# sleepybishop/nanorq

Measured on AMD Instinct MI355X. Metric: Gbit/s encode+decode, K=8192 T=1280, higher is better.
Workload: dtype u8

## Files before the change

__graft_entry__.py:

```python
import os
import sys

ROOT = os.path.dirname(os.path.abspath(__file__))
for p in (ROOT, os.path.join(ROOT, "tests")):
    if p not in sys.path:
        sys.path.insert(0, p)


def build():
    from nanorq_amd import build as nbuild
    nbuild.build_lib(verbose=True)
    nbuild.build_emu()
    nbuild.build_planner_emu()
    nbuild.build_ingest_emu()
    nbuild.build_emit_emu()
    nbuild.build_held_emu()
    nbuild.build_rxset_emu()
    nbuild.build_rxset_lists_emu()
    nbuild.build_txset_emu()
    nbuild.build_obj_emu()
    nbuild.build_shape_emu()
    nbuild.build_tools()
    import oracle
    oracle.build()
    if os.path.isfile("/root/reference/benchmark.c"):
        import subprocess
        subprocess.run(["make", "-s", "-C", os.path.join(ROOT, "oracle"), "_ref/benchmark_hip", "_ref/encode_hip", "_ref/decode_hip"],
                       check=True)
    import nanorq_amd
    nanorq_amd.lib()
    print("build ok:", nanorq_amd.lib_path())


def smoke():
    import numpy as np
# ... 29 lines not shown
```

nanorq_amd/binding.py:

```python
import ctypes as C
import os

import numpy as np

_HERE = os.path.dirname(os.path.abspath(__file__))
_LIB = None


class NrqError(RuntimeError):
    pass


class ObjParams(C.Structure):
    _fields_ = [("F", C.c_uint64)] + [(n, C.c_uint32) for n in
                                       ("T", "Al", "Z", "N", "Kt", "ZL", "KL", "KpL", "ZS", "KS", "KpS", "NL", "TL", "NS", "TS",
                                        "flags", "max_esi")] + [("oti_common", C.c_uint64), ("oti_specific", C.c_uint32)]

    def as_dict(self):
        return {n: getattr(self, n) for n, _ in self._fields_}


class CallStats(C.Structure):
    _fields_ = [("plan_ms", C.c_double), ("host_ms", C.c_double), ("strip_bytes", C.c_uint32),
                ("lds_bytes", C.c_uint32), ("grid", C.c_uint32), ("planner", C.c_uint32),
# ... 121 lines not shown
        L.nrq_rxset_decode.argtypes = [vp, ip, u32p]
    if hasattr(L, "nrq_txset_create"):
        L.nrq_txset_create.argtypes = [vp, C.c_uint32, C.POINTER(vp)]
        L.nrq_txset_destroy.argtypes = [vp]
        L.nrq_txset_destroy.restype = None
        L.nrq_txset_attach.argtypes = [vp, C.c_uint32, vp]
        L.nrq_txset_attach_obj.argtypes = [vp, C.c_uint32, vp]
        L.nrq_txset_detach.argtypes = [vp, C.c_uint32]
        L.nrq_txset_blocks.argtypes = [vp, u32p, u32p, C.c_uint32, u32p]
        L.nrq_txset_emit.argtypes = [vp, vp, vp, C.c_uint32, vp, sz, C.c_uint32, vp]
    u8pp = C.POINTER(C.POINTER(C.c_uint8))
    L.nrq_host_kconst_build.argtypes = [C.c_uint32, u8pp, u32p]
    L.nrq_host_plan_build.argtypes = [C.c_uint32, C.c_uint32, u32p, C.POINTER(C.c_uint8), u8pp, u32p]
    L.nrq_host_free.argtypes = [vp]
    L.nrq_host_free.restype = None
    _LIB = L
    return L


PARAM_NAMES = ("Kp", "J", "S", "H", "W", "L", "P", "P1", "U", "B")
PLAN_FIELDS = ("magic status K Kp J S H W L P P1 B M npiv u nlow r2 nfree nlev nrows pipe wpr "
               "npiv_pad n_xor_ops off_ops off_pivslot off_pivcol off_wt off_lowslot off_pivx off_fbits "
               "off_mh off_freex off_hinv off_colslot off_pivof off_uslot total_bytes reserved0 reserved1 fail_site "
               "off_augt lpr aug_stride nneed need_pad off_needslot off_wneed").split()


def params(K):
    out = (C.c_uint32 * 10)()
    if lib().nrq_params(K, out) != 0:
        raise ValueError("K out of range: %r" % (K,))
    return dict(zip(PARAM_NAMES, (int(x) for x in out)))


def _u32(a):
    return a.ctypes.data_as(C.POINTER(C.c_uint32))


def host_kconst(K):
    out = C.POINTER(C.c_uint8)()
    n = C.c_uint32()
    if lib().nrq_host_kconst_build(K, C.byref(out), C.byref(n)) != 0:
        raise NrqError("kconst build failed")
    buf = bytes(C.string_at(out, n.value))
    lib().nrq_host_free(out)
    return buf


# ... 664 lines not shown
```

nanorq_amd/build.py:

```python
import os
import shutil
import subprocess
import sys

HERE = os.path.dirname(os.path.abspath(__file__))
ROOT = os.path.dirname(HERE)
CSRC = os.path.join(HERE, "csrc")
LIB = os.path.join(HERE, "libnanorq_hip.so")
EMU = os.path.join(ROOT, "tests", "emu", "libsolve_emu.so")
PEMU = os.path.join(ROOT, "tests", "emu", "libplanner_emu.so")
IEMU = os.path.join(ROOT, "tests", "emu", "libingest_emu.so")
XEMU = os.path.join(ROOT, "tests", "emu", "libemit_emu.so")
OEMU = os.path.join(ROOT, "tests", "emu", "libobj_emu.so")
SEMU = os.path.join(ROOT, "tests", "emu", "libshape_emu.so")
HEMU = os.path.join(ROOT, "tests", "emu", "libheld_emu.so")
WEMU = os.path.join(ROOT, "tests", "emu", "libwant_emu.so")
REMU = os.path.join(ROOT, "tests", "emu", "librxset_emu.so")
LEMU = os.path.join(ROOT, "tests", "emu", "librxset_lists_emu.so")
TEMU = os.path.join(ROOT, "tests", "emu", "libtxset_emu.so")

HIP_SOURCES = ["nrq_device.hip"]
CXX_SOURCES = ["planner_host.cpp"]
C_SOURCES = ["nanorq_api.c", "io.c"]


def _hipcc():
    for c in (os.environ.get("HIPCC"), "/opt/rocm/bin/hipcc", shutil.which("hipcc")):
        if c and os.path.exists(c):
            return c
    raise RuntimeError("hipcc not found: the HIP extension cannot be built (no CPU fallback exists)")


def _newer(target, deps):
    if not os.path.exists(target):
        return True
    t = os.path.getmtime(target)
    return any(os.path.getmtime(d) > t for d in deps if os.path.exists(d))


def _deps():
    out = []
    for d in (CSRC, os.path.join(ROOT, "include")):
# ... 45 lines not shown
    return target


def build_tools(force=False):
    src = os.path.join(ROOT, "tools", "rqfile.c")
    exe = os.path.join(ROOT, "tools", "rqfile")
    deps = [src, LIB] + [os.path.join(ROOT, "include", h) for h in ("nanorq.h", "nanorq_batch.h", "io.h")]
    if force or _newer(exe, deps):
        subprocess.run(["gcc", "-std=c99", "-D_DEFAULT_SOURCE", "-D_FILE_OFFSET_BITS=64", "-O2", "-Wall", "-I" + os.path.join(ROOT, "include"),
                        src, "-o", exe, "-L" + os.path.dirname(LIB), "-lnanorq_hip", "-Wl,-rpath,$ORIGIN/../nanorq_amd", "-lm"], check=True)
    return exe


def _build_emu(target, src, headers, force):
    if force or _newer(target, [src] + [os.path.join(CSRC, h) for h in headers]):
        subprocess.run(["g++", "-O2", "-std=c++17", "-Wall", "-Wno-unknown-pragmas", "-fPIC", "-shared", "-o", target, src], check=True)
    return target


def build_emu(force=False):
    return _build_emu(EMU, os.path.join(ROOT, "tests", "emu", "solve_emu.cpp"), ("solve_body.h", "split_body.h", "plan.h", "rq_math.h"), force)


def build_planner_emu(force=False):
    return _build_emu(PEMU, os.path.join(ROOT, "tests", "emu", "planner_emu.cpp"),
                      ("planner_body.h", "planner_seq.h", "solve_body.h", "plan.h", "rq_math.h"), force)


def build_ingest_emu(force=False):
    return _build_emu(IEMU, os.path.join(ROOT, "tests", "emu", "ingest_emu.cpp"), ("ingest_body.h",), force)


def build_emit_emu(force=False):
    return _build_emu(XEMU, os.path.join(CSRC, "emit_emu.cpp"), ("emit_body.h", "rq_math.h"), force)


def build_held_emu(force=False):
    return _build_emu(HEMU, os.path.join(CSRC, "held_emu.cpp"), ("emit_body.h", "held_body.h", "ingest_body.h", "rq_math.h"), force)


def build_want_emu(force=False):
    return _build_emu(WEMU, os.path.join(CSRC, "want_emu.cpp"), ("want_body.h", "held_body.h", "ingest_body.h"), force)


def build_rxset_emu(force=False):
    return _build_emu(REMU, os.path.join(CSRC, "rxset_emu.cpp"), ("ingest_set_body.h", "ingest_body.h"), force)


def build_rxset_lists_emu(force=False):
    return _build_emu(LEMU, os.path.join(CSRC, "rxset_lists_emu.cpp"),
                      ("lists_set_body.h", "rxset_plan.h", "ingest_set_body.h", "ingest_body.h"), force)


def build_txset_emu(force=False):
    return _build_emu(TEMU, os.path.join(CSRC, "txset_emu.cpp"), ("emit_set_body.h", "emit_body.h", "rq_math.h"), force)


def build_obj_emu(force=False):
    return _build_emu(OEMU, os.path.join(ROOT, "tests", "emu", "obj_emu.cpp"), ("obj_body.h", "emit_body.h", "rq_math.h"), force)


def build_shape_emu(force=False):
    return _build_emu(SEMU, os.path.join(ROOT, "tests", "emu", "shape_emu.cpp"),
                      ("launch_shape.h", "planner_body.h", "solve_body.h", "plan.h", "rq_math.h", "rfc6330_tables.h"), force)


if __name__ == "__main__":
    build_lib(force="-f" in sys.argv, verbose=True)
    build_emu(force="-f" in sys.argv)
    build_planner_emu(force="-f" in sys.argv)
    build_ingest_emu(force="-f" in sys.argv)
    build_emit_emu(force="-f" in sys.argv)
    build_held_emu(force="-f" in sys.argv)
    build_want_emu(force="-f" in sys.argv)
    build_rxset_emu(force="-f" in sys.argv)
    build_rxset_lists_emu(force="-f" in sys.argv)
    build_txset_emu(force="-f" in sys.argv)
    build_obj_emu(force="-f" in sys.argv)
    build_shape_emu(force="-f" in sys.argv)
    build_tools(force="-f" in sys.argv)
```

nanorq_amd/csrc/nrq_device.hip:

```cpp
#include <hip/hip_runtime.h>

#include <algorithm>
#include <atomic>
#include <chrono>
#include <cstdarg>
#include <cstdio>
#include <cstdlib>
#include <cstring>
#include <deque>
#include <map>
#include <new>
#include <string>
#include <thread>
#include <vector>

#include "../../include/nanorq_hip.h"
#include "plan.h"
#include "planner_host.h"
#include "rq_math.h"
#include "solve_body.h"
#include "split_body.h"
#include "planner_body.h"
#include "ingest_body.h"
#include "ingest_set_body.h"
// ... 308 lines not shown
      __syncthreads();
      NRQ_MARK(c, 4);
      if (dense_fold_shared(VNT) || G > 1) {
        ph_hdpc_reduce<WB, G>(c, vt, VNT);
        __syncthreads();
      }
      NRQ_MARK(c, 5);
      ph_dense_free<WB, G, (NT == 64)>(c, vt, VNT);
      __syncthreads();
      NRQ_MARK(c, 6);
      ph_dense_cu<WB, G, (NT == 64)>(c, vt, VNT);
      __syncthreads();
      NRQ_STAMP(5);
      NRQ_STOP(4)
      if (ybuf) {
        NRQ_STAMP(6);
        NRQ_STAMP(7);
        ph_store_raw<WB, G>(c, ostage_cur + (size_t)sidx * ostage_stride + subl * WB, vt, VNT);
      } else {
        ph_tables<WB, G>(c, vt, VNT);
        __syncthreads();
        NRQ_STAMP(6);
        NRQ_STOP(5)
        ph_backsub<WB, G, (NT >= 512)>(c, vt, VNT);
        ph_park<WB, G>(c, vt, VNT);
        __syncthreads();
        NRQ_STAMP(7);
        NRQ_STOP(6)
        ph_store<WB, G, (NT >= 512)>(c, ostage_cur + (size_t)sidx * ostage_stride + subl * WB, vt, VNT);
      }
      __syncthreads();
      NRQ_STAMP(8);
#undef NRQ_STAMP
#undef NRQ_STOP
    }
    __syncthreads();
    qp = q;
    q = qn;
    buf ^= 1u;
  }
  if (qp < nslots) {
    GroupDst<WB> gp;
    const uint32_t units_p = group_dst(qp, gp) << lsub;
    pf_scatter_impl<WB, G, MPIPE, ALX>(gp, ostage0 + (size_t)(buf ^ 1u) * SPL * ostage_stride, ostage_stride, 0u, units_p, (tid) / G, (NT) / G, subl);
  }
}

enum {
#ifdef NRQ_PROF_INIT
  pl_tag_pl_init_a = 0,
  pl_tag_pl_init_b = 2,
  pl_tag_pl_scan_a = 4,
// ... 4307 lines not shown
```

nanorq_amd/csrc/plan.h:

```cpp
#ifndef NRQ_PLAN_H
#define NRQ_PLAN_H

#include <stdint.h>

#define NRQ_PLAN_MAGIC 0x4e525131u
#define NRQ_ROW 64u
#ifndef NRQ_PIPE
#define NRQ_PIPE 2u
#endif
#ifndef NRQ_RING_MULT
#define NRQ_RING_MULT 5u
#endif
#define NRQ_RING (NRQ_RING_MULT * 4u * (NRQ_PIPE + 1u))
#define NRQ_RING_MAX (2u * NRQ_RING)
#define NRQ_PAD_ROWS (2u * NRQ_RING_MAX + NRQ_PIPE + 4u)
#define NRQ_OP_INDEX(row, lane) ((((size_t)(row) >> 2) * NRQ_ROW + (size_t)(lane)) * 4u + ((size_t)(row) & 3u))
#define NRQ_OP_LANE_OF_INDEX(i) ((uint32_t)((i) >> 2) & (NRQ_ROW - 1u))
#define NRQ_STREAM_ROWS(rows) (((rows) + 3u) & ~3u)
#define NRQ_SCRATCH 64u
#define NRQ_OP(dst, src) (((uint32_t)(dst) + NRQ_SCRATCH) | (((uint32_t)(src) + NRQ_SCRATCH) << 16))
#define NRQ_NOP_AT(pos) (((uint32_t)(pos) & (NRQ_ROW - 1u)) * 0x10001u)
#define NRQ_OP_IS_NOP(op) (((op) & 0xFFFFu) < NRQ_SCRATCH)
#define NRQ_OP_DST(op) (((op) & 0xFFFFu) - NRQ_SCRATCH)
#define NRQ_OP_SRC(op) (((op) >> 16) - NRQ_SCRATCH)
#define NRQ_NOSLOT 0xFFFFu
#define NRQ_MAX_FREE 32u

#define NRQ_LANE_CLASSES 8u
// ... 13 lines not shown
NRQ_PLAN_FN uint32_t nrq_lane_place(uint32_t span, const uint32_t *ct, uint32_t d, uint32_t r) {
  const uint32_t cap = span * NRQ_LANE_CLASSES;
  if (r >= cap) {
    uint32_t o = r - cap;
    for (uint32_t e = 0; e < d; e++) o += ct[e] > cap ? ct[e] - cap : 0u;
    for (uint32_t e = 0; e < NRQ_LANE_CLASSES; e++) {
      const uint32_t holes = ct[e] < cap ? cap - ct[e] : 0u;
      if (o < holes) { d = e; r = ct[e] + o; break; }
      o -= holes;
    }
  }
  return (r >> 1) * 16u + 2u * d + (r & 1u);
}
#ifndef NRQ_EARLY_NARROW
#define NRQ_EARLY_NARROW 128u
#endif
#ifndef NRQ_MULTI_INACT
#define NRQ_MULTI_INACT 8u
#endif

#ifndef NRQ_AUG_MATRIX_MIN_L
#define NRQ_AUG_MATRIX_MIN_L 5000u
#endif
typedef struct nrq_plan_hdr {
  uint32_t magic;
  uint32_t status;
  uint32_t K, Kp, J, S, H, W, L, P, P1, B;
  uint32_t M;
  uint32_t npiv;
  uint32_t u;
  uint32_t nlow;
  uint32_t r2;
  uint32_t nfree;
  uint32_t nlev;
  uint32_t nrows;
  uint32_t pipe;
  uint32_t wpr;
  uint32_t npiv_pad;
  uint32_t n_xor_ops;

  uint32_t off_ops;
  uint32_t off_pivslot;
  uint32_t off_pivcol;
  uint32_t off_wt;
  uint32_t off_lowslot;
  uint32_t off_pivx;
  uint32_t off_fbits;
  uint32_t off_mh;
  uint32_t off_freex;
  uint32_t off_hinv;
  uint32_t off_colslot;
  uint32_t off_pivof;
  uint32_t off_uslot;
  uint32_t total_bytes;
  uint32_t reserved[2];
  uint32_t fail_site;
  uint32_t off_augt;
  uint32_t lpr;
  uint32_t aug_stride;
  uint32_t nneed;
  uint32_t need_pad;
  uint32_t off_needslot;
  uint32_t off_wneed;
} nrq_plan_hdr;
#ifdef __cplusplus
static_assert(sizeof(nrq_plan_hdr) <= 256u, "nrq_plan_hdr is read as a 256-byte prefix");
#endif

#define NRQ_CHEAD 16u
typedef struct nrq_kconst_hdr {
  uint32_t Kp, S, H, n;
  uint32_t off_g;
  uint32_t off_b12;
  uint32_t total_bytes;
  uint32_t L, W, P, nnz;
  uint32_t off_rptr;
  uint32_t off_cidx;
  uint32_t off_cptr;
  uint32_t off_ridx;
  uint32_t off_state;
  uint32_t off_gt;
  uint32_t off_erow;
  uint32_t off_chead;
} nrq_kconst_hdr;

#endif
```

nanorq_amd/csrc/planner_host.cpp:

```cpp
#include <algorithm>
#include <cstdlib>
#include <cstring>
#include <vector>

#include "plan.h"
#include "planner_host.h"
#include "rq_math.h"

namespace {

struct GF {
  uint8_t exp[510], log[256], inv[256];
  GF() {
    uint32_t x = 1;
    for (int e = 0; e < 255; e++) {
      exp[e] = (uint8_t)x;
      log[x] = (uint8_t)e;
      x <<= 1;
      if (x & 0x100) x ^= 0x11D;
    }
    for (int e = 255; e < 510; e++) exp[e] = exp[e - 255];
    log[0] = 0; inv[0] = 0;
    for (int v = 1; v < 256; v++) inv[v] = exp[255 - log[v]];
  }
// ... 96 lines not shown
    b12[c] = (uint8_t)(b1 | (b2 << 4));
  }
  memcpy(buf + h.off_rptr, rptr.data(), (size_t)(L + 1) * 4);
  memcpy(buf + h.off_cidx, cidx.data(), (size_t)nnz * 2);
  memcpy(buf + h.off_cptr, cptr.data(), (size_t)(L + 1) * 4);
  memcpy(buf + h.off_ridx, ridx.data(), (size_t)nnz * 2);
  memcpy(buf + h.off_state, state.data(), (size_t)L * 4);
  for (uint32_t c = 0; c < L; c++)
    for (uint32_t q = 0; q < NRQ_CHEAD; q++)
      reinterpret_cast<uint16_t *>(buf + h.off_chead)[(size_t)c * NRQ_CHEAD + q] = cptr[c] + q < cptr[c + 1] ? ridx[cptr[c] + q] : (uint16_t)0xFFFFu;
  for (uint32_t r = 0; r < L; r++)
    for (uint32_t e = rptr[r]; e < rptr[r + 1]; e++) reinterpret_cast<uint16_t *>(buf + h.off_erow)[e] = (uint16_t)r;
  for (uint32_t c = 0; c < n; c++)
    for (uint32_t r = 0; r < H; r++) buf[h.off_gt + (size_t)c * 16 + r] = G[(size_t)r * n + c];
  memcpy(buf, &h, sizeof(h));
  *out = buf;
  *out_bytes = off;
  return 0;
}

extern "C" void nrq_host_free(void *p) { free(p); }

static int host_plan_build_with(uint32_t K, uint32_t nrows, const uint32_t *isis, const uint8_t *kconst, uint8_t **out, uint32_t *out_bytes,
                                uint32_t comp_rows) {
  rq_params p;
  if (!rq_params_init(K, &p)) return -1;
  if (nrows < p.Kp) return -1;
  const nrq_kconst_hdr *kh = reinterpret_cast<const nrq_kconst_hdr *>(kconst);
  if (!kh || kh->Kp != p.Kp) return -1;
  const uint8_t *G = kconst + kh->off_g;
  const uint32_t S = p.S, H = p.H, W = p.W, L = p.L, n_hd = p.Kp + p.S;
  const uint32_t M = S + H + nrows;
  if (M > 65535u) return -3;

  std::vector<uint32_t> rptr(M + 1, 0);
  std::vector<uint16_t> cidx;
  {
    const uint32_t *brp = reinterpret_cast<const uint32_t *>(kconst + kh->off_rptr);
    const uint16_t *bci = reinterpret_cast<const uint16_t *>(kconst + kh->off_cidx);
    cidx.reserve((size_t)kh->nnz + (size_t)(nrows - p.Kp + 8u) * RQ_MAX_LT_COLS);
    for (uint32_t r = 0; r < S; r++) {
      rptr[r] = (uint32_t)cidx.size();
      cidx.insert(cidx.end(), bci + brp[r], bci + brp[r + 1]);
    }
    for (uint32_t r = S; r < S + H; r++) rptr[r] = (uint32_t)cidx.size();
    uint32_t tmp[RQ_MAX_LT_COLS];
    for (uint32_t k = 0; k < nrows; k++) {
// ... 402 lines not shown
        for (uint32_t w = 0; w < aw; w++) aug[(size_t)h * aw + w] ^= gf.mul(b, aug[(size_t)pr * aw + w]);
      }
    }
    if (!status)
      for (uint32_t f = 0; f < nfree; f++)
        for (uint32_t h = 0; h < H; h++) hinv[(size_t)f * H + h] = aug[(size_t)solver[f] * aw + nfree + h];
  }

  std::vector<uint16_t> colslot(L, NRQ_NOSLOT), pivof(n_hd, NRQ_NOSLOT), uslot(u, NRQ_NOSLOT);
  for (uint32_t k = 0; k < npiv; k++) {
    colslot[pivcol[k]] = pivslot[k];
    pivof[pivcol[k]] = pivslot[k];
  }
  {
    uint32_t x = 0;
    for (uint32_t r = 0; r < M && x < u; r++)
      if (!assigned[r]) { uslot[x] = (uint16_t)r; colslot[ucol[x]] = (uint16_t)r; x++; }
    if (x != u) return -5;
  }

  Arena A;
  nrq_plan_hdr hd;
  memset(&hd, 0, sizeof(hd));
  A.buf.reserve(ops.size() * 4u + (size_t)wpr * ((npiv + 63u) & ~63u) * 4u + (size_t)L * 16u + (size_t)augt.size() * 4u + 8192u);
  A.reserve((uint32_t)sizeof(hd));
  hd.magic = NRQ_PLAN_MAGIC; hd.status = status;
  hd.K = K; hd.Kp = p.Kp; hd.J = p.J; hd.S = S; hd.H = H; hd.W = W; hd.L = L; hd.P = p.P; hd.P1 = p.P1; hd.B = p.B;
  hd.M = M; hd.npiv = npiv; hd.u = u; hd.nlow = nlow; hd.r2 = r2; hd.nfree = nfree; hd.nlev = nlev;
  hd.nrows = op_rows; hd.pipe = NRQ_PIPE; hd.wpr = wpr;
  hd.npiv_pad = (npiv + 63u) & ~63u;
  hd.n_xor_ops = n_real_ops;
  {
    while ((ops.size() / NRQ_ROW) % 4u) pad_rows(1);
    hd.off_ops = A.reserve((uint32_t)(ops.size() * 4));
    uint32_t *out = A.at<uint32_t>(hd.off_ops);
    const size_t nquads = ops.size() / (4u * NRQ_ROW);
    for (size_t g = 0; g < nquads; g++) {
      const uint32_t *r0 = &ops[g * 4u * NRQ_ROW];
      uint32_t *o = out + g * 4u * NRQ_ROW;
      for (uint32_t l = 0; l < NRQ_ROW; l++) {
        o[4u * l] = r0[l]; o[4u * l + 1u] = r0[NRQ_ROW + l]; o[4u * l + 2u] = r0[2u * NRQ_ROW + l]; o[4u * l + 3u] = r0[3u * NRQ_ROW + l];
      }
    }
  }
  hd.off_pivslot = A.reserve(npiv * 2);
  memcpy(A.at<uint8_t>(hd.off_pivslot), pivslot.data(), (size_t)npiv * 2);
  hd.off_pivcol = A.reserve(npiv * 2);
  memcpy(A.at<uint8_t>(hd.off_pivcol), pivcol.data(), (size_t)npiv * 2);
  hd.off_wt = A.reserve(wpr * hd.npiv_pad * 4);
  {
    uint32_t *wt = A.at<uint32_t>(hd.off_wt);
    for (uint32_t k = 0; k < npiv; k++)
      for (uint32_t w = 0; w < wpr; w++) wt[(size_t)w * hd.npiv_pad + k] = Wm[(size_t)k * wpr + w];
  }
  hd.off_lowslot = A.reserve(std::max(1u, nlow) * 2);
  if (nlow) memcpy(A.at<uint8_t>(hd.off_lowslot), lowslot.data(), (size_t)nlow * 2);
  hd.off_pivx = A.reserve(std::max(1u, r2) * 2);
  for (uint32_t q = 0; q < r2; q++) A.at<uint16_t>(hd.off_pivx)[q] = (uint16_t)red_x[q];
  hd.off_fbits = A.reserve(std::max(1u, r2) * 4);
  memcpy(A.at<uint8_t>(hd.off_fbits), fbits.data(), (size_t)std::max(1u, r2) * 4);
  hd.off_mh = A.reserve(H * std::max(1u, r2));
  memcpy(A.at<uint8_t>(hd.off_mh), mh.data(), (size_t)H * std::max(1u, r2));
  hd.off_freex = A.reserve(std::max(1u, nfree) * 2);
  for (uint32_t f = 0; f < nfree; f++) A.at<uint16_t>(hd.off_freex)[f] = (uint16_t)freex[f];
  hd.off_hinv = A.reserve(std::max(1u, nfree) * H);
  memcpy(A.at<uint8_t>(hd.off_hinv), hinv.data(), (size_t)std::max(1u, nfree) * H);
  hd.off_colslot = A.reserve(L * 2);
  memcpy(A.at<uint8_t>(hd.off_colslot), colslot.data(), (size_t)L * 2);
  hd.off_pivof = A.reserve(n_hd * 2);
  memcpy(A.at<uint8_t>(hd.off_pivof), pivof.data(), (size_t)n_hd * 2);
  hd.off_uslot = A.reserve(std::max(1u, u) * 2);
  if (u) memcpy(A.at<uint8_t>(hd.off_uslot), uslot.data(), (size_t)u * 2);
  hd.lpr = aug_in_stream ? 0u : lpr; hd.aug_stride = aug_stride;
  hd.off_augt = A.reserve((uint32_t)(augt.size() * 4 + 16));
  if (!augt.empty()) memcpy(A.at<uint8_t>(hd.off_augt), augt.data(), augt.size() * 4);
  hd.total_bytes = align16((uint32_t)A.buf.size());
  A.buf.resize(hd.total_bytes, 0);
  memcpy(A.buf.data(), &hd, sizeof(hd));

  uint8_t *res = (uint8_t *)malloc(hd.total_bytes);
  if (!res) return -2;
  memcpy(res, A.buf.data(), hd.total_bytes);
  *out = res;
  *out_bytes = hd.total_bytes;
  return 0;
}

extern "C" int nrq_host_plan_build(uint32_t K, uint32_t nrows, const uint32_t *isis, const uint8_t *kconst, uint8_t **out, uint32_t *out_bytes) {
  rq_params p;
  if (!rq_params_init(K, &p)) return -1;
  bool encoder = nrows == p.Kp;
  for (uint32_t k = 0; encoder && k < nrows; k++) encoder = isis[k] == k;
  uint32_t way = !encoder ? 0u : p.Kp >= 1500u ? 1u : 6u;
  if (const char *e = getenv("NRQ_HOST_WAY")) { if (encoder) way = (uint32_t)atoi(e); }
  return host_plan_build_with(K, nrows, isis, kconst, out, out_bytes, way);
}
```

nanorq_amd/csrc/solve_body.h:

```cpp
#ifndef NRQ_SOLVE_BODY_H
#define NRQ_SOLVE_BODY_H

#include <stdint.h>
#include <string.h>

#include "plan.h"

#if defined(__HIPCC__)
#define SB_HD __host__ __device__ __forceinline__
#define SB_MEM __host__ __device__ __forceinline__
#else
#define SB_HD static inline
#define SB_MEM inline
struct uint2 { uint32_t x, y; };
struct uint4 { uint32_t x, y, z, w; };
#endif

#if defined(__HIP_DEVICE_COMPILE__)
#define NRQ_GAS __attribute__((address_space(1)))
#else
#define NRQ_GAS
#endif
template <class X> SB_HD const NRQ_GAS X *gptr(const void *p) { return (const NRQ_GAS X *)p; }
template <class X> SB_HD const NRQ_GAS X *gptr(uint64_t p) { return (const NRQ_GAS X *)(uintptr_t)p; }
// ... 335 lines not shown
      typedef uint32_t u4 __attribute__((ext_vector_type(4)));
      const u4 t = {v.w[0], v.w[1], v.w[2], v.w[3]};
      __builtin_nontemporal_store(t, reinterpret_cast<NRQ_GAS u4 *>(p));
    } else if constexpr (WB == 12) {
      typedef uint32_t u3 __attribute__((ext_vector_type(3)));
      typedef u3 u3a __attribute__((aligned(4)));
      const u3 t = {v.w[0], v.w[1], v.w[2]};
      __builtin_nontemporal_store(t, reinterpret_cast<NRQ_GAS u3a *>(p));
    } else if constexpr (WB == 8) {
      typedef uint32_t u2 __attribute__((ext_vector_type(2)));
      const u2 t = {v.w[0], v.w[1]};
      __builtin_nontemporal_store(t, reinterpret_cast<NRQ_GAS u2 *>(p));
    } else if constexpr (WB == 4) {
      __builtin_nontemporal_store(v.w[0], reinterpret_cast<NRQ_GAS uint32_t *>(p));
    } else {
      __builtin_nontemporal_store((uint16_t)v.w[0], reinterpret_cast<NRQ_GAS uint16_t *>(p));
    }
    return;
  }
#endif
  g_put<WB>(p, valid, v);
}

typedef struct nrq_lds_layout {
  uint32_t off_slots, off_cu, off_x, total;
} nrq_lds_layout;

SB_HD uint32_t nrq_r16(uint32_t x) { return (x + 15u) & ~15u; }

SB_HD nrq_lds_layout nrq_lds_plan(const nrq_plan_hdr *h, uint32_t WB) {
  nrq_lds_layout l;
  uint32_t o = 0;
  o = NRQ_SCRATCH * WB;
  l.off_slots = o; o = nrq_r16(o + (h->M + h->r2) * WB);
  l.off_cu = o;    o = nrq_r16(o + (h->u ? h->u : 1u) * WB);
  uint32_t cf = NRQ_MAX_FREE * WB;
  uint32_t t4 = h->wpr * 8u * 16u * (WB == 12u ? 16u : WB);
  l.off_x = o;
  o = nrq_r16(o + (cf > t4 ? cf : t4));
  l.total = o;
  return l;
}

template <int WB, int G = 1> struct StripCtx {
  const uint8_t *plan;
  const nrq_plan_hdr *h;
// ... 857 lines not shown
  if constexpr (WB == 12) {
    uint4 t; t.x = v.w[0]; t.y = v.w[1]; t.z = v.w[2]; t.w = 0u;
    reinterpret_cast<uint4 *>(t4)[e] = t;
  } else lds_put<WB, G>(t4, e, v);
}
template <int WB, int G = 1> SB_HD void ph_tables(const StripCtx<WB, G> &c, uint32_t tid, uint32_t nt) {
  const uint32_t ngroups = c.h->wpr * 8u, u = c.h->u;
  for (uint32_t e = tid; e < ngroups * 16u; e += nt) {
    uint32_t grp = e >> 4, nib = e & 15u;
    SV<WB> v = sv_zero<WB>();
#pragma unroll
    for (uint32_t bq = 0; bq < 4; bq++) {
      uint32_t x = grp * 4u + bq;
      if (((nib >> bq) & 1u) && x < u) {
        SV<WB> t = lds_get<WB, G>(c.cu(), x);
        sv_xor<WB>(v, t);
      }
    }
    t4_put<WB, G>(c.t4(), e, v);
  }
}

template <int WB, int NW, int G = 1, bool FAST = true>
SB_HD void backsub_one(const StripCtx<WB, G> &c, const uint8_t *t4, uint32_t slot, const uint32_t (&bitsw)[NW],
                       uint32_t wpr) {
  SV<WB> acc = lds_get<WB, G>(c.slots(), slot);
#pragma unroll
  for (uint32_t w = 0; w < (uint32_t)NW; w++) {
    if (w >= wpr) break;
    const uint32_t bits = bitsw[w];
#if defined(__HIP_DEVICE_COMPILE__)
    if constexpr (WB == 16 && G == 1) {
      uint32_t odd = bits & 0xF0F0F0F0u, even = (bits << 4) & 0xF0F0F0F0u;
      asm volatile("" : "+v"(odd), "+v"(even));
      if constexpr (FAST) {
      const uint32_t tbw = (uint32_t)(uintptr_t)t4 + w * 2048u;
      uint4 d[8];
#pragma unroll
      for (uint32_t q = 0; q < 8; q++) d[q] = *NRQ_LDSP(uint4, t4_addr(tbw, (q & 1u) ? odd : even, q >> 1) + q * 256u);
#pragma unroll
      for (uint32_t q = 0; q < 8; q += 2) {
        acc.w[0] = nrq_xor3(acc.w[0], d[q].x, d[q + 1].x); acc.w[1] = nrq_xor3(acc.w[1], d[q].y, d[q + 1].y);
        acc.w[2] = nrq_xor3(acc.w[2], d[q].z, d[q + 1].z); acc.w[3] = nrq_xor3(acc.w[3], d[q].w, d[q + 1].w);
      }
      } else {
        const uint32_t tb = (uint32_t)(uintptr_t)t4;
#pragma unroll
      for (uint32_t q = 0; q < 8; q++) {
        const uint32_t a = t4_addr(tb, (q & 1u) ? odd : even, q >> 1) + (w * 8u + q) * 256u;
// ... 26 lines not shown
      uint4 d[8];
#pragma unroll
      for (uint32_t q = 0; q < 8; q++) d[q] = *NRQ_LDSP(uint4, t4_addr(tbw, (q & 1u) ? odd : even, q >> 1) + q * 256u);
      uint32_t pad = 0;
#pragma unroll
      for (uint32_t q = 0; q < 8; q += 2) {
        acc.w[0] = nrq_xor3(acc.w[0], d[q].x, d[q + 1].x); acc.w[1] = nrq_xor3(acc.w[1], d[q].y, d[q + 1].y);
        acc.w[2] = nrq_xor3(acc.w[2], d[q].z, d[q + 1].z); pad = nrq_xor3(pad, d[q].w, d[q + 1].w);
      }
      asm volatile("" : : "v"(pad));
      NRQ_SCHED_FENCE();
      continue;
    }
#endif
#pragma unroll
    for (uint32_t q = 0; q < 8; q++) {
      const uint32_t nib = (bits >> (4u * q)) & 15u;
      SV<WB> t = t4_get<WB, G>(t4, (w * 8u + q) * 16u + nib);
      sv_xor<WB>(acc, t);
      if (q == 3) NRQ_SCHED_FENCE();
    }
    NRQ_SCHED_FENCE();
  }
  lds_put<WB, G>(c.slots(), slot, acc);
}

#define NRQ_BACKSUB_VIEW(c, need)                                                                                            \
  const NRQ_GAS uint16_t *pivslot = (c).template arr<uint16_t>((need) ? (c).h->off_needslot : (c).h->off_pivslot);      \
  const NRQ_GAS uint32_t *wt = (c).template arr<uint32_t>((need) ? (c).h->off_wneed : (c).h->off_wt);                   \
  const uint32_t stride = (need) ? (c).h->need_pad : (c).h->npiv_pad, npiv = (need) ? (c).h->nneed : (c).h->npiv
template <int WB, int NW, int G = 1, bool FAST = true>
SB_HD void backsub_fixed(const StripCtx<WB, G> &c, bool need, uint32_t tid, uint32_t nt) {
  if constexpr (!FAST) {

  NRQ_BACKSUB_VIEW(c, need);
  const uint32_t wpr = c.h->wpr;
  const uint8_t *t4 = c.t4();
  for (uint32_t k = tid; k < npiv; k += 2 * nt) {
    const uint32_t k2 = k + nt;
    uint32_t a[NW], b[NW];
    const uint32_t sa = pivslot[k];
    const uint32_t sb = k2 < npiv ? pivslot[k2] : 0u;
#pragma unroll
    for (uint32_t w = 0; w < (uint32_t)NW; w++) a[w] = w < wpr ? wt[(size_t)w * stride + k] : 0u;
#pragma unroll
    for (uint32_t w = 0; w < (uint32_t)NW; w++) b[w] = (w < wpr && k2 < npiv) ? wt[(size_t)w * stride + k2] : 0u;
    backsub_one<WB, NW, G, false>(c, t4, sa, a, wpr);
    if (k2 < npiv) backsub_one<WB, NW, G, false>(c, t4, sb, b, wpr);
  }
    return;
  }
  NRQ_BACKSUB_VIEW(c, need);
  const uint32_t wpr = c.h->wpr;
  const uint8_t *t4 = c.t4();
  uint32_t a[NW], b[NW], sa = 0, sb = 0;
  uint32_t k = tid;
  if (k < npiv) {
    sa = pivslot[k];
#pragma unroll
    for (uint32_t w = 0; w < (uint32_t)NW; w++) a[w] = w < wpr ? wt[(size_t)w * stride + k] : 0u;
  }
  for (; k < npiv; k += 2 * nt) {
    const uint32_t k2 = k + nt, k3 = k + 2 * nt;
    if (k2 < npiv) {
      sb = pivslot[k2];
#pragma unroll
      for (uint32_t w = 0; w < (uint32_t)NW; w++) b[w] = w < wpr ? wt[(size_t)w * stride + k2] : 0u;
    }
    backsub_one<WB, NW, G, FAST>(c, t4, sa, a, wpr);
    if (k3 < npiv) {
      sa = pivslot[k3];
#pragma unroll
      for (uint32_t w = 0; w < (uint32_t)NW; w++) a[w] = w < wpr ? wt[(size_t)w * stride + k3] : 0u;
    }
    if (k2 < npiv) backsub_one<WB, NW, G, FAST>(c, t4, sb, b, wpr);
  }
}

template <int WB, int G = 1, bool FAST = true> SB_HD void ph_backsub(const StripCtx<WB, G> &c, uint32_t tid, uint32_t nt) {
  const uint32_t wpr = c.h->wpr;
  const bool need = c.job->inter == 0 && c.h->off_needslot != 0u;
  if (wpr <= 4) backsub_fixed<WB, 4, G, FAST>(c, need, tid, nt);
  else if (wpr <= 8) backsub_fixed<WB, 8, G, FAST>(c, need, tid, nt);
  else if (wpr <= 12) backsub_fixed<WB, 12, G, FAST>(c, need, tid, nt);
  else if (wpr <= 24) backsub_fixed<WB, 24, G, FAST>(c, need, tid, nt);
  else {
    NRQ_BACKSUB_VIEW(c, need);
    const uint8_t *t4 = c.t4();
    for (uint32_t k = tid; k < npiv; k += nt) {
      uint32_t s = pivslot[k];
      SV<WB> acc = lds_get<WB, G>(c.slots(), s);
      for (uint32_t w = 0; w < wpr; w++) {
        uint32_t bits = wt[(size_t)w * stride + k];
#pragma unroll
        for (uint32_t q = 0; q < 8; q++) {
          uint32_t nib = (bits >> (4u * q)) & 15u;
          SV<WB> t = t4_get<WB, G>(t4, (w * 8u + q) * 16u + nib);
          sv_xor<WB>(acc, t);
        }
      }
      lds_put<WB, G>(c.slots(), s, acc);
    }
  }
}

template <int WB, int G = 1> SB_HD void ph_park(const StripCtx<WB, G> &c, uint32_t tid, uint32_t nt) {
  const NRQ_GAS uint16_t *uslot = c.template arr<uint16_t>(c.h->off_uslot);
  for (uint32_t x = tid; x < c.h->u; x += nt) lds_put<WB, G>(c.slots(), uslot[x], lds_get<WB, G>(c.cu(), x));
}

#ifndef NRQ_STORE_CHUNK
#define NRQ_STORE_CHUNK 8u
#endif
#ifndef NRQ_STORE_TRIP
#define NRQ_STORE_TRIP 32u
#endif
#define NRQ_STORE_SLACK (16u + NRQ_STORE_TRIP * 4u)
#define NRQ_LT_LIST_MAX 33u
static_assert(NRQ_LT_LIST_MAX <= 2u * NRQ_STORE_TRIP, "ph_store reads at most two trips of a list; out_slots[] slack is sized for that");
template <int WB, int G = 1> SB_HD uint32_t out_elems(const nrq_job *job, const nrq_plan_hdr *h) { return (job->inter ? h->L : 0u) + job->nout; }
SB_HD void store_trip(const NRQ_GAS uint16_t *osl, uint32_t e, uint32_t end, uint32_t (&raw)[NRQ_STORE_TRIP / 2u]) {
  (void)end;
#ifdef __HIP_DEVICE_COMPILE__
  typedef uint32_t u4 __attribute__((ext_vector_type(4)));
  typedef u4 u4a __attribute__((aligned(2)));
#pragma unroll
  for (uint32_t k = 0; k < NRQ_STORE_TRIP / 8u; k++) {
    const u4 w = *reinterpret_cast<const NRQ_GAS u4a *>(osl + e + 8u * k);
    raw[4u * k] = w.x; raw[4u * k + 1u] = w.y; raw[4u * k + 2u] = w.z; raw[4u * k + 3u] = w.w;
  }
#else
#pragma unroll
  for (uint32_t k = 0; k < NRQ_STORE_TRIP / 2u; k++)
    raw[k] = (e + 2u * k < end ? (uint32_t)osl[e + 2u * k] : 0u) | (e + 2u * k + 1u < end ? (uint32_t)osl[e + 2u * k + 1u] : 0u) << 16;
#endif
}
SB_HD uint32_t store_slot(const uint32_t (&raw)[NRQ_STORE_TRIP / 2u], uint32_t k, uint32_t e, uint32_t end, uint32_t zero_at) {
  return e + k < end ? ((raw[k / 2u] >> (16u * (k & 1u))) & 0xFFFFu) + NRQ_SCRATCH : zero_at;
}
template <int WB, int G = 1, bool FAST = true> SB_HD void ph_store(const StripCtx<WB, G> &c, NRQ_GAS uint8_t *ostage, uint32_t tid, uint32_t nt) {
  constexpr int STB = 8;
  const NRQ_GAS uint16_t *colslot = c.template arr<uint16_t>(c.h->off_colslot);
  const uint32_t L = c.h->L, ni = c.job->inter ? L : 0u;
  for (uint32_t base = tid; base < ni; base += STB * nt) {
    uint32_t sl[STB];
#pragma unroll
    for (int q = 0; q < STB; q++) {
      uint32_t col = base + (uint32_t)q * nt;
      sl[q] = col < L ? colslot[col] : 0u;
    }
#pragma unroll
    for (int q = 0; q < STB; q++) {
      uint32_t col = base + (uint32_t)q * nt;
      if (col < L) g_put_stream<WB>(ostage + (size_t)col * (WB * G), WB, lds_get<WB, G>(c.slots(), sl[q]));
    }
  }
  const NRQ_GAS uint32_t *cptr = gptr<uint32_t>(c.job->out_cptr);
  const NRQ_GAS uint16_t *osl = gptr<uint16_t>(c.job->out_slots);
  if constexpr (FAST) {
  const uint32_t nout = c.job->nout;
  constexpr uint32_t CH = NRQ_STORE_CHUNK;
  const uint32_t zero_at = tid & (NRQ_SCRATCH - 1u);
  uint32_t e_n = 0, end_n = 0;
  if (tid < nout) { e_n = cptr[tid]; end_n = cptr[tid + 1]; }
  const uint32_t npass = (nout + nt - 1u) / nt;
  for (uint32_t pass = 0, q = tid; pass < npass; pass++, q += nt) {
    uint32_t e = e_n;
    const uint32_t end = end_n;
    e_n = end_n = 0;
    if (q + nt < nout) { e_n = cptr[q + nt]; end_n = cptr[q + nt + 1]; }
    SV<WB> acc = sv_zero<WB>();
    while (NRQ_WAVE_ANY(e < end)) {
      constexpr uint32_t TR = NRQ_STORE_TRIP;
      uint32_t raw[TR / 2u];
      store_trip(osl, e, end, raw);
#pragma unroll
      for (uint32_t k0 = 0; k0 < TR; k0 += CH) {
        if (k0 && !NRQ_WAVE_ANY(e + k0 < end)) break;
        SV<WB> v[CH];
// ... 157 lines not shown
```

Measured before the change: 1620.

## Fuse intermediate-symbol stores into back-substitution and park via column-ordered view

Adds a column-ordered view to the encoder plan, holding pivot entries packed as slot|col<<16, a matching reordered weight table and the u-column list. With this view, back-substitution and park write each intermediate symbol straight to the output stage with non-temporal stores as soon as it is computed. The separate copy pass over L columns in ph_store is then skipped. The aim is to drop one full LDS-read-plus-global-write sweep and to spread the stores across the compute phase. The cost is a larger plan and more scattered global writes during back-substitution.

```diff
diff --git a/__graft_entry__.py b/__graft_entry__.py
--- a/__graft_entry__.py
+++ b/__graft_entry__.py
@@ -11,6 +11,7 @@
     from nanorq_amd import build as nbuild
     nbuild.build_lib(verbose=True)
     nbuild.build_emu()
+    nbuild.build_colview_emu()
     nbuild.build_planner_emu()
     nbuild.build_ingest_emu()
     nbuild.build_emit_emu()
diff --git a/nanorq_amd/binding.py b/nanorq_amd/binding.py
--- a/nanorq_amd/binding.py
+++ b/nanorq_amd/binding.py
@@ -167,7 +167,8 @@
 PLAN_FIELDS = ("magic status K Kp J S H W L P P1 B M npiv u nlow r2 nfree nlev nrows pipe wpr "
                "npiv_pad n_xor_ops off_ops off_pivslot off_pivcol off_wt off_lowslot off_pivx off_fbits "
                "off_mh off_freex off_hinv off_colslot off_pivof off_uslot total_bytes reserved0 reserved1 fail_site "
-               "off_augt lpr aug_stride nneed need_pad off_needslot off_wneed").split()
+               "off_augt lpr aug_stride nneed need_pad off_needslot off_wneed "
+               "off_cv").split()
 
 
 def params(K):
diff --git a/nanorq_amd/build.py b/nanorq_amd/build.py
--- a/nanorq_amd/build.py
+++ b/nanorq_amd/build.py
@@ -18,6 +18,7 @@
 REMU = os.path.join(ROOT, "tests", "emu", "librxset_emu.so")
 LEMU = os.path.join(ROOT, "tests", "emu", "librxset_lists_emu.so")
 TEMU = os.path.join(ROOT, "tests", "emu", "libtxset_emu.so")
+CEMU = os.path.join(ROOT, "tests", "emu", "libcolview_emu.so")
 
 HIP_SOURCES = ["nrq_device.hip"]
 CXX_SOURCES = ["planner_host.cpp"]
@@ -109,6 +110,11 @@
     return _build_emu(EMU, os.path.join(ROOT, "tests", "emu", "solve_emu.cpp"), ("solve_body.h", "split_body.h", "plan.h", "rq_math.h"), force)
 
 
+def build_colview_emu(force=False):
+    return _build_emu(CEMU, os.path.join(ROOT, "tests", "emu", "colview_emu.cpp"),
+                      ("solve_body.h", "split_body.h", "plan.h", "rq_math.h", os.path.join(ROOT, "tests", "emu", "solve_emu.cpp")), force)
+
+
 def build_planner_emu(force=False):
     return _build_emu(PEMU, os.path.join(ROOT, "tests", "emu", "planner_emu.cpp"),
                       ("planner_body.h", "planner_seq.h", "solve_body.h", "plan.h", "rq_math.h"), force)
@@ -155,6 +161,7 @@
 if __name__ == "__main__":
     build_lib(force="-f" in sys.argv, verbose=True)
     build_emu(force="-f" in sys.argv)
+    build_colview_emu(force="-f" in sys.argv)
     build_planner_emu(force="-f" in sys.argv)
     build_ingest_emu(force="-f" in sys.argv)
     build_emit_emu(force="-f" in sys.argv)
diff --git a/nanorq_amd/csrc/nrq_device.hip b/nanorq_amd/csrc/nrq_device.hip
--- a/nanorq_amd/csrc/nrq_device.hip
+++ b/nanorq_amd/csrc/nrq_device.hip
@@ -354,12 +354,13 @@
         __syncthreads();
         NRQ_STAMP(6);
         NRQ_STOP(5)
-        ph_backsub<WB, G, (NT >= 512)>(c, vt, VNT);
-        ph_park<WB, G>(c, vt, VNT);
+        NRQ_GAS uint8_t *const ost = ostage_cur + (size_t)sidx * ostage_stride + subl * WB;
+        ph_backsub<WB, G, (NT >= 512)>(c, ost, vt, VNT);
+        ph_park<WB, G>(c, ost, vt, VNT);
         __syncthreads();
         NRQ_STAMP(7);
         NRQ_STOP(6)
-        ph_store<WB, G, (NT >= 512)>(c, ostage_cur + (size_t)sidx * ostage_stride + subl * WB, vt, VNT);
+        ph_store<WB, G, (NT >= 512), true>(c, ost, vt, VNT);
       }
       __syncthreads();
       NRQ_STAMP(8);
diff --git a/nanorq_amd/csrc/plan.h b/nanorq_amd/csrc/plan.h
--- a/nanorq_amd/csrc/plan.h
+++ b/nanorq_amd/csrc/plan.h
@@ -3,7 +3,7 @@
 
 #include <stdint.h>
 
-#define NRQ_PLAN_MAGIC 0x4e525131u
+#define NRQ_PLAN_MAGIC 0x4e525132u
 #define NRQ_ROW 64u
 #ifndef NRQ_PIPE
 #define NRQ_PIPE 2u
@@ -63,6 +63,9 @@
 #ifndef NRQ_AUG_MATRIX_MIN_L
 #define NRQ_AUG_MATRIX_MIN_L 5000u
 #endif
+#ifndef NRQ_COLVIEW_MIN_L
+#define NRQ_COLVIEW_MIN_L 0u
+#endif
 typedef struct nrq_plan_hdr {
   uint32_t magic;
   uint32_t status;
@@ -103,7 +106,11 @@
   uint32_t need_pad;
   uint32_t off_needslot;
   uint32_t off_wneed;
+  uint32_t off_cv;
 } nrq_plan_hdr;
+#define NRQ_CV_WOFF(off_cv, npiv_pad) ((off_cv) + (npiv_pad) * 4u)
+#define NRQ_CV_UOFF(off_cv, npiv_pad, wpr) ((off_cv) + (npiv_pad) * 4u * (1u + (wpr)))
+#define NRQ_CV_BYTES(npiv_pad, wpr, u) ((npiv_pad) * 4u * (1u + (wpr)) + (u) * 2u)
 #ifdef __cplusplus
 static_assert(sizeof(nrq_plan_hdr) <= 256u, "nrq_plan_hdr is read as a 256-byte prefix");
 #endif
diff --git a/nanorq_amd/csrc/planner_host.cpp b/nanorq_amd/csrc/planner_host.cpp
--- a/nanorq_amd/csrc/planner_host.cpp
+++ b/nanorq_amd/csrc/planner_host.cpp
@@ -142,7 +142,7 @@
 extern "C" void nrq_host_free(void *p) { free(p); }
 
 static int host_plan_build_with(uint32_t K, uint32_t nrows, const uint32_t *isis, const uint8_t *kconst, uint8_t **out, uint32_t *out_bytes,
-                                uint32_t comp_rows) {
+                                uint32_t comp_rows, bool colview) {
   rq_params p;
   if (!rq_params_init(K, &p)) return -1;
   if (nrows < p.Kp) return -1;
@@ -591,7 +591,7 @@
   Arena A;
   nrq_plan_hdr hd;
   memset(&hd, 0, sizeof(hd));
-  A.buf.reserve(ops.size() * 4u + (size_t)wpr * ((npiv + 63u) & ~63u) * 4u + (size_t)L * 16u + (size_t)augt.size() * 4u + 8192u);
+  A.buf.reserve(ops.size() * 4u + (size_t)wpr * ((npiv + 63u) & ~63u) * (colview ? 8u : 4u) + (size_t)L * 24u + (size_t)augt.size() * 4u + 8192u);
   A.reserve((uint32_t)sizeof(hd));
   hd.magic = NRQ_PLAN_MAGIC; hd.status = status;
   hd.K = K; hd.Kp = p.Kp; hd.J = p.J; hd.S = S; hd.H = H; hd.W = W; hd.L = L; hd.P = p.P; hd.P1 = p.P1; hd.B = p.B;
@@ -617,10 +617,32 @@
   hd.off_pivcol = A.reserve(npiv * 2);
   memcpy(A.at<uint8_t>(hd.off_pivcol), pivcol.data(), (size_t)npiv * 2);
   hd.off_wt = A.reserve(wpr * hd.npiv_pad * 4);
-  {
-    uint32_t *wt = A.at<uint32_t>(hd.off_wt);
-    for (uint32_t k = 0; k < npiv; k++)
-      for (uint32_t w = 0; w < wpr; w++) wt[(size_t)w * hd.npiv_pad + k] = Wm[(size_t)k * wpr + w];
+  std::vector<uint32_t> cvpos;
+  if (colview) {
+    hd.off_cv = A.reserve(NRQ_CV_BYTES(hd.npiv_pad, wpr, u));
+    if (u) memcpy(A.at<uint8_t>(NRQ_CV_UOFF(hd.off_cv, hd.npiv_pad, wpr)), ucol.data(), (size_t)u * 2);
+    cvpos.assign(npiv, 0);
+    std::vector<uint32_t> kofcol(L, 0xFFFFFFFFu);
+    for (uint32_t k = 0; k < npiv; k++) kofcol[pivcol[k]] = k;
+    uint32_t *ce = A.at<uint32_t>(hd.off_cv);
+    uint32_t e = 0;
+    for (uint32_t col = 0; col < L; col++) {
+      const uint32_t k = kofcol[col];
+      if (k == 0xFFFFFFFFu) continue;
+      ce[e] = (uint32_t)pivslot[k] | col << 16; cvpos[k] = e++;
+    }
+    if (e != npiv) return -5;
+  }
+  {
+    uint32_t *wt = A.at<uint32_t>(hd.off_wt), *wcv = colview ? A.at<uint32_t>(NRQ_CV_WOFF(hd.off_cv, hd.npiv_pad)) : nullptr;
+    for (uint32_t k = 0; k < npiv; k++) {
+      const uint32_t *row = &Wm[(size_t)k * wpr];
+      for (uint32_t w = 0; w < wpr; w++) wt[(size_t)w * hd.npiv_pad + k] = row[w];
+      if (wcv) {
+        const uint32_t e = cvpos[k];
+        for (uint32_t w = 0; w < wpr; w++) wcv[(size_t)w * hd.npiv_pad + e] = row[w];
+      }
+    }
   }
   hd.off_lowslot = A.reserve(std::max(1u, nlow) * 2);
   if (nlow) memcpy(A.at<uint8_t>(hd.off_lowslot), lowslot.data(), (size_t)nlow * 2);
@@ -662,5 +684,5 @@
   for (uint32_t k = 0; encoder && k < nrows; k++) encoder = isis[k] == k;
   uint32_t way = !encoder ? 0u : p.Kp >= 1500u ? 1u : 6u;
   if (const char *e = getenv("NRQ_HOST_WAY")) { if (encoder) way = (uint32_t)atoi(e); }
-  return host_plan_build_with(K, nrows, isis, kconst, out, out_bytes, way);
+  return host_plan_build_with(K, nrows, isis, kconst, out, out_bytes, way, encoder && p.L >= NRQ_COLVIEW_MIN_L);
 }
diff --git a/nanorq_amd/csrc/solve_body.h b/nanorq_amd/csrc/solve_body.h
--- a/nanorq_amd/csrc/solve_body.h
+++ b/nanorq_amd/csrc/solve_body.h
@@ -381,6 +381,32 @@
   g_put<WB>(p, valid, v);
 }
 
+template <int WB> SB_HD void g_put_stage(NRQ_GAS uint8_t *stage, uint32_t off, const SV<WB> &v) {
+#if defined(__HIP_DEVICE_COMPILE__)
+  NRQ_GAS uint8_t *p = stage + off;
+  if constexpr (WB == 16) {
+    typedef uint32_t u4 __attribute__((ext_vector_type(4)));
+    const u4 t = {v.w[0], v.w[1], v.w[2], v.w[3]};
+    __builtin_nontemporal_store(t, reinterpret_cast<NRQ_GAS u4 *>(p));
+  } else if constexpr (WB == 12) {
+    typedef uint32_t u3 __attribute__((ext_vector_type(3)));
+    typedef u3 u3a __attribute__((aligned(4)));
+    const u3 t = {v.w[0], v.w[1], v.w[2]};
+    __builtin_nontemporal_store(t, reinterpret_cast<NRQ_GAS u3a *>(p));
+  } else if constexpr (WB == 8) {
+    typedef uint32_t u2 __attribute__((ext_vector_type(2)));
+    const u2 t = {v.w[0], v.w[1]};
+    __builtin_nontemporal_store(t, reinterpret_cast<NRQ_GAS u2 *>(p));
+  } else if constexpr (WB == 4) {
+    __builtin_nontemporal_store(v.w[0], reinterpret_cast<NRQ_GAS uint32_t *>(p));
+  } else {
+    __builtin_nontemporal_store((uint16_t)v.w[0], reinterpret_cast<NRQ_GAS uint16_t *>(p));
+  }
+#else
+  g_put<WB>(stage + off, WB, v);
+#endif
+}
+
 typedef struct nrq_lds_layout {
   uint32_t off_slots, off_cu, off_x, total;
 } nrq_lds_layout;
@@ -1284,9 +1310,9 @@
 }
 
 template <int WB, int NW, int G = 1, bool FAST = true>
-SB_HD void backsub_one(const StripCtx<WB, G> &c, const uint8_t *t4, uint32_t slot, const uint32_t (&bitsw)[NW],
-                       uint32_t wpr) {
-  SV<WB> acc = lds_get<WB, G>(c.slots(), slot);
+SB_HD void backsub_one(const StripCtx<WB, G> &c, const uint8_t *t4, uint32_t ent, const uint32_t (&bitsw)[NW],
+                       uint32_t wpr, bool cv = false, NRQ_GAS uint8_t *ostage = nullptr) {
+  SV<WB> acc = lds_get<WB, G>(c.slots(), ent & 0xFFFFu);
 #pragma unroll
   for (uint32_t w = 0; w < (uint32_t)NW; w++) {
     if (w >= wpr) break;
@@ -1359,73 +1385,79 @@
     }
     NRQ_SCHED_FENCE();
   }
-  lds_put<WB, G>(c.slots(), slot, acc);
-}
-
-#define NRQ_BACKSUB_VIEW(c, need)                                                                                            \
+  lds_put<WB, G>(c.slots(), ent & 0xFFFFu, acc);
+  if (cv) g_put_stage<WB>(ostage, (ent >> 16) * (uint32_t)(WB * G), acc);
+}
+
+SB_HD bool backsub_colview(const nrq_job *job, const nrq_plan_hdr *h) { return job->inter != 0 && h->off_cv != 0u; }
+#define NRQ_BACKSUB_VIEW(c, need, cv)                                                                                        \
   const NRQ_GAS uint16_t *pivslot = (c).template arr<uint16_t>((need) ? (c).h->off_needslot : (c).h->off_pivslot);      \
-  const NRQ_GAS uint32_t *wt = (c).template arr<uint32_t>((need) ? (c).h->off_wneed : (c).h->off_wt);                   \
+  const NRQ_GAS uint32_t *cvent = (c).template arr<uint32_t>((c).h->off_cv);                                          \
+  const NRQ_GAS uint32_t *wt = (c).template arr<uint32_t>((cv) ? NRQ_CV_WOFF((c).h->off_cv, (c).h->npiv_pad) : (need) ? (c).h->off_wneed : (c).h->off_wt); \
   const uint32_t stride = (need) ? (c).h->need_pad : (c).h->npiv_pad, npiv = (need) ? (c).h->nneed : (c).h->npiv
+#define NRQ_BACKSUB_ENT(k) ((cv) ? cvent[k] : (uint32_t)pivslot[k])
 template <int WB, int NW, int G = 1, bool FAST = true>
-SB_HD void backsub_fixed(const StripCtx<WB, G> &c, bool need, uint32_t tid, uint32_t nt) {
+SB_HD void backsub_fixed(const StripCtx<WB, G> &c, bool need, bool cv, NRQ_GAS uint8_t *ostage, uint32_t tid, uint32_t nt) {
   if constexpr (!FAST) {
 
-  NRQ_BACKSUB_VIEW(c, need);
+  NRQ_BACKSUB_VIEW(c, need, cv);
   const uint32_t wpr = c.h->wpr;
   const uint8_t *t4 = c.t4();
   for (uint32_t k = tid; k < npiv; k += 2 * nt) {
     const uint32_t k2 = k + nt;
     uint32_t a[NW], b[NW];
-    const uint32_t sa = pivslot[k];
-    const uint32_t sb = k2 < npiv ? pivslot[k2] : 0u;
+    const uint32_t sa = NRQ_BACKSUB_ENT(k);
+    const uint32_t sb = k2 < npiv ? NRQ_BACKSUB_ENT(k2) : 0u;
 #pragma unroll
     for (uint32_t w = 0; w < (uint32_t)NW; w++) a[w] = w < wpr ? wt[(size_t)w * stride + k] : 0u;
 #pragma unroll
     for (uint32_t w = 0; w < (uint32_t)NW; w++) b[w] = (w < wpr && k2 < npiv) ? wt[(size_t)w * stride + k2] : 0u;
-    backsub_one<WB, NW, G, false>(c, t4, sa, a, wpr);
-    if (k2 < npiv) backsub_one<WB, NW, G, false>(c, t4, sb, b, wpr);
+    backsub_one<WB, NW, G, false>(c, t4, sa, a, wpr, cv, ostage);
+    if (k2 < npiv) backsub_one<WB, NW, G, false>(c, t4, sb, b, wpr, cv, ostage);
   }
     return;
   }
-  NRQ_BACKSUB_VIEW(c, need);
+  NRQ_BACKSUB_VIEW(c, need, cv);
   const uint32_t wpr = c.h->wpr;
   const uint8_t *t4 = c.t4();
   uint32_t a[NW], b[NW], sa = 0, sb = 0;
   uint32_t k = tid;
   if (k < npiv) {
-    sa = pivslot[k];
+    sa = NRQ_BACKSUB_ENT(k);
 #pragma unroll
     for (uint32_t w = 0; w < (uint32_t)NW; w++) a[w] = w < wpr ? wt[(size_t)w * stride + k] : 0u;
   }
   for (; k < npiv; k += 2 * nt) {
     const uint32_t k2 = k + nt, k3 = k + 2 * nt;
     if (k2 < npiv) {
-      sb = pivslot[k2];
+      sb = NRQ_BACKSUB_ENT(k2);
 #pragma unroll
       for (uint32_t w = 0; w < (uint32_t)NW; w++) b[w] = w < wpr ? wt[(size_t)w * stride + k2] : 0u;
     }
-    backsub_one<WB, NW, G, FAST>(c, t4, sa, a, wpr);
+    backsub_one<WB, NW, G, FAST>(c, t4, sa, a, wpr, cv, ostage);
     if (k3 < npiv) {
-      sa = pivslot[k3];
+      sa = NRQ_BACKSUB_ENT(k3);
 #pragma unroll
       for (uint32_t w = 0; w < (uint32_t)NW; w++) a[w] = w < wpr ? wt[(size_t)w * stride + k3] : 0u;
     }
-    if (k2 < npiv) backsub_one<WB, NW, G, FAST>(c, t4, sb, b, wpr);
-  }
-}
-
-template <int WB, int G = 1, bool FAST = true> SB_HD void ph_backsub(const StripCtx<WB, G> &c, uint32_t tid, uint32_t nt) {
+    if (k2 < npiv) backsub_one<WB, NW, G, FAST>(c, t4, sb, b, wpr, cv, ostage);
+  }
+}
+
+template <int WB, int G = 1, bool FAST = true>
+SB_HD void ph_backsub(const StripCtx<WB, G> &c, NRQ_GAS uint8_t *ostage, uint32_t tid, uint32_t nt) {
   const uint32_t wpr = c.h->wpr;
   const bool need = c.job->inter == 0 && c.h->off_needslot != 0u;
-  if (wpr <= 4) backsub_fixed<WB, 4, G, FAST>(c, need, tid, nt);
-  else if (wpr <= 8) backsub_fixed<WB, 8, G, FAST>(c, need, tid, nt);
-  else if (wpr <= 12) backsub_fixed<WB, 12, G, FAST>(c, need, tid, nt);
-  else if (wpr <= 24) backsub_fixed<WB, 24, G, FAST>(c, need, tid, nt);
+  const bool cv = ostage && backsub_colview(c.job, c.h);
+  if (wpr <= 4) backsub_fixed<WB, 4, G, FAST>(c, need, cv, ostage, tid, nt);
+  else if (wpr <= 8) backsub_fixed<WB, 8, G, FAST>(c, need, cv, ostage, tid, nt);
+  else if (wpr <= 12) backsub_fixed<WB, 12, G, FAST>(c, need, cv, ostage, tid, nt);
+  else if (wpr <= 24) backsub_fixed<WB, 24, G, FAST>(c, need, cv, ostage, tid, nt);
   else {
-    NRQ_BACKSUB_VIEW(c, need);
+    NRQ_BACKSUB_VIEW(c, need, cv);
     const uint8_t *t4 = c.t4();
     for (uint32_t k = tid; k < npiv; k += nt) {
-      uint32_t s = pivslot[k];
+      const uint32_t ent = NRQ_BACKSUB_ENT(k), s = ent & 0xFFFFu;
       SV<WB> acc = lds_get<WB, G>(c.slots(), s);
       for (uint32_t w = 0; w < wpr; w++) {
         uint32_t bits = wt[(size_t)w * stride + k];
@@ -1437,14 +1469,30 @@
         }
       }
       lds_put<WB, G>(c.slots(), s, acc);
-    }
-  }
-}
-
-template <int WB, int G = 1> SB_HD void ph_park(const StripCtx<WB, G> &c, uint32_t tid, uint32_t nt) {
+      if (cv) g_put_stage<WB>(ostage, (ent >> 16) * (uint32_t)(WB * G), acc);
+    }
+  }
+}
+
+template <int WB, int G = 1, bool FAST = true> SB_HD void ph_backsub(const StripCtx<WB, G> &c, uint32_t tid, uint32_t nt) {
+  ph_backsub<WB, G, FAST>(c, nullptr, tid, nt);
+}
+
+template <int WB, int G = 1> SB_HD void ph_park(const StripCtx<WB, G> &c, NRQ_GAS uint8_t *ostage, uint32_t tid, uint32_t nt) {
   const NRQ_GAS uint16_t *uslot = c.template arr<uint16_t>(c.h->off_uslot);
+  if (ostage && backsub_colview(c.job, c.h)) {
+    const NRQ_GAS uint16_t *ucol = c.template arr<uint16_t>(NRQ_CV_UOFF(c.h->off_cv, c.h->npiv_pad, c.h->wpr));
+    for (uint32_t x = tid; x < c.h->u; x += nt) {
+      const SV<WB> v = lds_get<WB, G>(c.cu(), x);
+      lds_put<WB, G>(c.slots(), uslot[x], v);
+      g_put_stage<WB>(ostage, (uint32_t)ucol[x] * (uint32_t)(WB * G), v);
+    }
+    return;
+  }
   for (uint32_t x = tid; x < c.h->u; x += nt) lds_put<WB, G>(c.slots(), uslot[x], lds_get<WB, G>(c.cu(), x));
 }
+
+template <int WB, int G = 1> SB_HD void ph_park(const StripCtx<WB, G> &c, uint32_t tid, uint32_t nt) { ph_park<WB, G>(c, nullptr, tid, nt); }
 
 #ifndef NRQ_STORE_CHUNK
 #define NRQ_STORE_CHUNK 8u
@@ -1475,11 +1523,14 @@
 SB_HD uint32_t store_slot(const uint32_t (&raw)[NRQ_STORE_TRIP / 2u], uint32_t k, uint32_t e, uint32_t end, uint32_t zero_at) {
   return e + k < end ? ((raw[k / 2u] >> (16u * (k & 1u))) & 0xFFFFu) + NRQ_SCRATCH : zero_at;
 }
-template <int WB, int G = 1, bool FAST = true> SB_HD void ph_store(const StripCtx<WB, G> &c, NRQ_GAS uint8_t *ostage, uint32_t tid, uint32_t nt) {
+template <int WB, int G = 1, bool FAST = true, bool CV = false>
+SB_HD void ph_store(const StripCtx<WB, G> &c, NRQ_GAS uint8_t *ostage, uint32_t tid, uint32_t nt) {
   constexpr int STB = 8;
   const NRQ_GAS uint16_t *colslot = c.template arr<uint16_t>(c.h->off_colslot);
   const uint32_t L = c.h->L, ni = c.job->inter ? L : 0u;
-  for (uint32_t base = tid; base < ni; base += STB * nt) {
+  const uint32_t ncopy = (CV && backsub_colview(c.job, c.h)) ? 0u : ni;
+#ifndef NRQ_EXPERIMENT_NO_INTER_STORE
+  for (uint32_t base = tid; base < ncopy; base += STB * nt) {
     uint32_t sl[STB];
 #pragma unroll
     for (int q = 0; q < STB; q++) {
@@ -1492,6 +1543,7 @@
       if (col < L) g_put_stream<WB>(ostage + (size_t)col * (WB * G), WB, lds_get<WB, G>(c.slots(), sl[q]));
     }
   }
+#endif
   const NRQ_GAS uint32_t *cptr = gptr<uint32_t>(c.job->out_cptr);
   const NRQ_GAS uint16_t *osl = gptr<uint16_t>(c.job->out_slots);
   if constexpr (FAST) {
```

Result: no change. 1625, median of 6 (+0.3%).
